# jrnerupudinho/Semi-Blind-Channel-Estimation-for-MIMO-RIS-communication-system-Using-EM-Algo

Measured on AMD Instinct MI355X. Metric: EM-iterations/sec (whole node) + NMSE@SNR; Nt=Nr=4, N_RIS=64, Tp=16 Td=256, higher is better.
Workload: dtype f64; 1 GPU; cfg1; n_tx=4, n_rx=4, N_RIS=64, T_p=16, T_d=256, M=16, trials_per_gpu=1000, em_iters=20, estep=soft, partition_r=0, solve=chol, parallelism=trials-sharded x1, streams_per_gpu=3

## Files before the change

semi-blind-channel-estimation-for-mimo-ris-communication-system-using-em-algo_amd/csrc/api.hip:

```cpp
#include <stdlib.h>
#include <string.h>

#include <atomic>
#include <initializer_list>
#include <mutex>
#include <vector>

#include "sbce_internal.h"

using namespace sbce;

namespace sbce {

#if SBCE_AB
DebugConfig g_debug;

namespace {
void read_debug_env(DebugConfig& c) {
    c = kDebugDefault;
    auto env = [](const char* n) { const char* v = getenv(n); return (v && v[0]) ? v : nullptr; };
    const char* v;
    if ((v = env("SBCE_ESTEP_IMPL"))) c.estep_valu = v[0] == 'v';
    if ((v = env("SBCE_ESTEP_PRUNE"))) c.estep_noprune = v[0] == '0';
    if ((v = env("SBCE_ESTEP_COUNT"))) c.estep_count = v[0] == '1';
    if ((v = env("SBCE_ESTEP_F32"))) c.estep_nof32 = v[0] == '0';
    if ((v = env("SBCE_ESTEP_SPHERE"))) c.estep_nosphere = v[0] == '0';
    if ((v = env("SBCE_SPHERE_BUDGET"))) {
        const int bu = atoi(v);
        c.sphere_budget = bu < 1 ? 1 : (bu > kBfsPmax ? kBfsPmax : bu);
    }
    if ((v = env("SBCE_BACKSUB"))) c.backsub_general = v[0] == '1';
    if ((v = env("SBCE_CHOL_IMPL"))) c.chol_valu = v[0] == 'v';
    if ((v = env("SBCE_ESTEP_PAIR"))) c.estep_nopair = v[0] == '0';
    if ((v = env("SBCE_CPLX3"))) c.cplx3 = v[0] != '0';
    if ((v = env("SBCE_MSTEP_SMALL"))) {
        c.mstep_nosmall = v[0] == '0';
        c.small_valu = v[0] == 'v';
        c.small_v1 = v[0] == '1';
    }
    if ((v = env("SBCE_PM_IMPL"))) c.pm_impl = (v[0] == 'w' || v[0] == 't' || v[0] == 'q') ? v[0] : 0;
    if ((v = env("SBCE_SMALL_SOLVE"))) c.small_col = v[0] == 'c';
    if ((v = env("SBCE_ESTEP_TRI"))) c.estep_tri = (v[0] >= '0' && v[0] <= '2') ? v[0] - '0' : 1;
    if ((v = env("SBCE_SMALL_STOP"))) c.small_stop = (v[0] >= '1' && v[0] <= '4') ? v[0] - '0' : 0;
}

__attribute__((constructor)) void load_debug_env() { read_debug_env(g_debug); }
}

bool debug_nondefault() {
    const DebugConfig& c = g_debug;
    const DebugConfig& d = kDebugDefault;
    return c.estep_valu != d.estep_valu || c.estep_noprune != d.estep_noprune ||
           c.estep_nof32 != d.estep_nof32 || c.estep_tri != d.estep_tri ||
           c.estep_nosphere != d.estep_nosphere || c.sphere_budget != d.sphere_budget ||
           c.backsub_general != d.backsub_general || c.chol_valu != d.chol_valu ||
           c.estep_nopair != d.estep_nopair || c.cplx3 != d.cplx3 ||
           c.mstep_nosmall != d.mstep_nosmall || c.small_stop != d.small_stop ||
           c.small_valu != d.small_valu || c.small_v1 != d.small_v1 || c.small_col != d.small_col ||
           (chol_debug_skip_mask() & 31);
}
#else
bool debug_nondefault() { return false; }
#endif

}

namespace {

constexpr size_t kAlign = 256;
size_t align_up(size_t v) { return (v + kAlign - 1) / kAlign * kAlign; }

struct Carve {
    size_t mom, R, rhs, done, mchg, ysh, prep, list, tree, tol, winv, ppsi, pS, pflag, prhs, gram, grhs,
        act, tol2, dvec, mnr, mnskip, total;
    bool has_prep, has_prhs, has_winv, has_mn;
};

constexpr int kAnySolve = -1;

bool make_problem(const sbce_dims* d, Problem& pb) {
    if (!d) return false;
    if (d->batch < 0 || d->n_tx < 1 || d->n_rx < 1 || d->n_psi < 1 || d->t_p < 0 || d->t_d < 1 ||
        d->m < 2 || d->partition_r < 0 || !(d->varn > 0.0))
        return false;
    if (d->n_tx > 8 || d->n_rx > 8) return false;
    pb.B = d->batch; pb.NT = d->n_tx; pb.NR = d->n_rx; pb.P = d->n_psi;
    pb.Tp = d->t_p; pb.Td = d->t_d; pb.M = d->m; pb.varn = d->varn; pb.pr = d->partition_r;
    pb.varx = d->varx;
    pb.L = pb.P * pb.NT;
    pb.K = pb.L * pb.NR;
    return true;
}

Carve carve(const Problem& pb, int solve = kAnySolve) {
    Carve c;
    const size_t MS = (size_t)pb.NT + (size_t)pb.NT * pb.NT;
    c.mom = 0;
    c.R = align_up(c.mom + (size_t)pb.B * pb.Td * MS * sizeof(cd));
    c.rhs = align_up(c.R + (size_t)pb.B * pb.L * pb.L * sizeof(cd));
    c.done = align_up(c.rhs + (size_t)pb.B * pb.L * pb.NR * sizeof(cd));
    c.ysh = align_up(c.done + (size_t)pb.B * sizeof(int32_t));
    c.mchg = c.ysh;
    c.prep = align_up(c.ysh + (size_t)pb.B * pb.Td * pb.NR * sizeof(cd));
    const int ps = estep_prep_stride(pb);
    c.has_prep = ps > 0;
    c.list = align_up(c.prep + (size_t)pb.B * pb.Td * ps * sizeof(double));
    c.tree = align_up(c.list + (3 * (size_t)pb.B * pb.Td + 2 * kEstepListCnt) * sizeof(int32_t));
    c.tol = c.has_prep ? align_up(c.tree + (size_t)pb.B * pb.Td * kTreeRecDoubles * sizeof(double))
                       : c.list;
    c.ppsi = c.pS = c.pflag = c.winv = c.tol;
    c.total = c.tol;
    if (rbuild_herm_supported(pb)) {
        c.ppsi = c.total;
        c.pS = align_up(c.ppsi + (size_t)pb.B * pb.Tp * pb.P * sizeof(cd));
        c.pflag = align_up(c.pS + (size_t)pb.B * pb.Tp * pb.NT * pb.NT * sizeof(cd));
        c.total = align_up(c.pflag + (size_t)pb.B * sizeof(int32_t));
    }
    c.has_prhs = rbuild_herm_supported(pb) && pb.L <= kLargeL;
    c.prhs = c.total;
    if (c.has_prhs) c.total = align_up(c.prhs + (size_t)pb.B * pb.L * pb.NR * sizeof(cd));
    c.tol = c.total;
    c.winv = align_up(c.tol + (size_t)pb.B * sizeof(double));
    c.total = c.winv;
    c.has_mn = solve == kAnySolve || solve == SBCE_SOLVE_MINNORM;
    c.has_winv = c.has_mn || pb.L > kLargeL;
    c.gram = c.winv;
    if (c.has_winv) c.total = c.gram = align_up(c.winv + (size_t)pb.B * 64 * 64 * sizeof(cd));
    c.grhs = c.act = c.tol2 = c.dvec = c.mnr = c.mnskip = c.total;
    if (c.has_mn) {
        c.grhs = align_up(c.gram + (size_t)pb.B * pb.L * pb.L * sizeof(cd));
        c.act = align_up(c.grhs + (size_t)pb.B * pb.L * pb.NR * sizeof(cd));
        c.tol2 = align_up(c.act + (size_t)pb.B * sizeof(int32_t));
        c.dvec = align_up(c.tol2 + (size_t)pb.B * sizeof(double));
        c.mnr = align_up(c.dvec + (size_t)pb.B * pb.L * sizeof(double));
        c.mnskip = align_up(c.mnr + (size_t)pb.B * pb.L * pb.NR * sizeof(cd));
        c.total = align_up(c.mnskip + (size_t)pb.B * sizeof(int32_t));
// ... 926 lines not shown
```

semi-blind-channel-estimation-for-mimo-ris-communication-system-using-em-algo_amd/csrc/estep_sweep.hip:

```cpp
#include "sbce_internal.h"

namespace sbce {

namespace {


template <int NT, int NR>
__device__ double candidate_distance(const cd* H, const cd* yg, const cd* s_cons, int M,
                                     double reg, cd* scratch, int lane, double& scale) {
    cd* sG = scratch;
    cd* sHy = scratch + 16;
    if (lane < NT * NT) {
        const int u = lane / NT, v = lane - u * NT;
        cd acc = czero();
#pragma unroll
        for (int r = 0; r < NR; ++r) acc = cfmac(acc, H[v * NR + r], H[u * NR + r]);
        if (u == v) acc.x += reg;
        sG[lane] = acc;
    } else if (lane >= 32 && lane < 32 + NT) {
        const int u = lane - 32;
        cd acc = czero();
#pragma unroll
        for (int r = 0; r < NR; ++r) acc = cfmac(acc, yg[r], H[u * NR + r]);
        sHy[u] = acc;
// ... 19 lines not shown
    }
#pragma unroll
    for (int i = 0; i < NT; ++i) {
        cd s = sHy[i];
#pragma unroll
        for (int k = 0; k < i; ++k) s = csub(s, cmul(Lm[i][k], z[k]));
        z[i] = cscale(s, dinv[i]);
    }
#pragma unroll
    for (int i = NT - 1; i >= 0; --i) {
        cd s = z[i];
#pragma unroll
        for (int k = i + 1; k < NT; ++k) s = csub(s, cmul(cconj(Lm[k][i]), z[k]));
        z[i] = cscale(s, dinv[i]);
    }
    const int qa = lane >> 4;
    cd za = z[0];
#pragma unroll
    for (int q = 1; q < NT; ++q) za = csel(qa == q, z[q], za);
    double bd = INFINITY;
    int bs = 0;
    if (qa < NT)
        for (int s = lane & 15; s < M; s += 16) {
            const double dd = cabs2(csub(za, s_cons[s]));
            if (dd < bd) { bd = dd; bs = s; }
        }
    for (int off = 8; off >= 1; off >>= 1) {
        const double od = shfl_xor_d(bd, off);
        const int os = __shfl_xor(bs, off);
        if (od < bd || (od == bd && os < bs)) { bd = od; bs = os; }
    }
    cd x[NT];
#pragma unroll
    for (int q = 0; q < NT; ++q) x[q] = s_cons[__shfl(bs, 16 * q)];
    double d0 = 0.0, sc = 0.0;
#pragma unroll
    for (int r = 0; r < NR; ++r) {
        cd res = yg[r];
        sc += cabs2(res);
#pragma unroll
        for (int q = 0; q < NT; ++q) {
            const cd hx = cmul(H[q * NR + r], x[q]);
            res = csub(res, hx);
            sc += NT * cabs2(hx);
        }
        d0 += cabs2(res);
    }
    wave_sync();
    scale = sc;
    return d0;
}


constexpr int kMfmaWaves = 2;
constexpr int kChunk = 256;
constexpr int kScreenD = 256;

typedef float f4v __attribute__((ext_vector_type(4)));

constexpr int mfma_rec_d(int rec_words) { return 2 * (rec_words <= 128 ? 160 : (rec_words + 1) / 2 * 2 + 32); }
constexpr int mfma_tri_d(int steps) { return 3 * 64 * steps / 2 + 128; }
constexpr int mfma_tab_d(int NO, int chunk, int steps, int M, int nkt_pad, int rec_words) {
    return (2 * NO + chunk + 3 * (4 * steps) * M + nkt_pad + 128 + 1) / 2 * 2 + mfma_rec_d(rec_words) +
           kScreenD + (M == 16 && chunk == 256 ? mfma_tri_d(steps) : 0);
}
constexpr int kTriGate = 4;

struct MfmaConst {
    int B, Td, P, M, lm;
    int JA, JB, chunk, nparts;
    int tab_d;
    double inv_s2, thr_d;
    double reg;
    int nkt_pad;
    int prune;
    int count;
    int prep_stride;
    int rowb_off;
    int rowb;
    int rec_words;
    int spw;
    int screen;
    int tri;
};

template <int NT, int NR>
__device__ double column_tile_bounds(const cd* H, const cd* yg, const cd* s_cons, int M, int lm,
                                     int nkt, double* s_lb, cd* scratch, int lane) {
    constexpr int NA = NT / 2, NB = NT - NA;
    const int mask = M - 1;
    const int r = lane & 7;
    const bool own = r < NR;
    int xa[6];
#pragma unroll
    for (int i = 0; i < 6; ++i) xa[i] = (lane ^ (32 >> i)) << 2;
    auto rsum = [&](double v) {
#pragma unroll
        for (int i = 3; i < 6; ++i) v += bperm_d(v, xa[i]);
        return v;
    };
    auto rdot = [&](cd u, cd v) { return cmk(rsum(fma(v.x, u.x, v.y * u.y)),
                                             rsum(fma(v.y, u.x, -v.x * u.y))); };
    cd u[NA];
    bool ok = true;
#pragma unroll
    for (int q = 0; q < NA; ++q) {
        cd v = own ? H[q * NR + r] : czero();
        const double h2 = rsum(cabs2(v));
#pragma unroll
        for (int rep = 0; rep < 2; ++rep)
#pragma unroll
            for (int j = 0; j < q; ++j) v = csub(v, cmul(u[j], rdot(u[j], v)));
        const double n2 = rsum(cabs2(v));
        ok = ok && h2 > 0.0 && n2 > 1e-6 * h2;
        u[q] = cscale(v, ok ? fast_rsqrt(n2) : 0.0);
    }
    cd w = own ? yg[r] : czero();
    double sc = rsum(cabs2(w));
    cd g[NB];
    double g2 = 0.0;
#pragma unroll
    for (int b = 0; b < NB; ++b) {
        g[b] = own ? H[(NA + b) * NR + r] : czero();
        g2 += cabs2(g[b]);
    }
#pragma unroll
    for (int j = 0; j < NA; ++j) {
        w = csub(w, cmul(u[j], rdot(u[j], w)));
#pragma unroll
        for (int b = 0; b < NB; ++b) g[b] = csub(g[b], cmul(u[j], rdot(u[j], g[b])));
    }
    if (lane < NR) {
        scratch[r] = w;
#pragma unroll
        for (int b = 0; b < NB; ++b) scratch[8 * (b + 1) + r] = g[b];
    }
    double cmax2 = lane < M ? cabs2(s_cons[lane]) : 0.0;
#pragma unroll
    for (int i = 0; i < 6; ++i) cmax2 = fmax(cmax2, bperm_d(cmax2, xa[i]));
    sc += NB * cmax2 * rsum(g2);
    wave_sync();
    for (int kt0 = 0; kt0 < nkt; kt0 += 4) {
        const int kt = kt0 + (lane >> 4);
        const int k = kt * 16 + (lane & 15);
        cd xb[NB];
#pragma unroll
        for (int b = 0; b < NB; ++b) xb[b] = s_cons[(k >> (lm * (NB - 1 - b))) & mask];
        double lb = 0.0;
#pragma unroll
        for (int rr = 0; rr < NR; ++rr) {
            cd res = scratch[rr];
#pragma unroll
            for (int b = 0; b < NB; ++b) res = csub(res, cmul(scratch[8 * (b + 1) + rr], xb[b]));
            lb += cabs2(res);
        }
        if (!ok) lb = 0.0;
#pragma unroll
        for (int i = 2; i < 6; ++i) lb = fmin(lb, bperm_d(lb, xa[i]));
        if ((lane & 15) == 0 && kt < nkt) s_lb[kt] = lb;
    }
    wave_sync();
    return sc;
}

__device__ unsigned long long g_estep_mfma;
__device__ unsigned long long g_estep_groups;
// ... 284 lines not shown
        for (int pass = 0; pass < 2; ++pass) {
            const int q = pass ? 1 : 3, o = pass ? 3 : 1;
            const cd hq = own ? H[q * NR + r] : czero();
            const cd v = own ? (vi == 0 ? yv[r] : H[(vi == 1 ? 0 : (vi == 2 ? o : 2)) * NR + r]) : czero();
            const double hq2 = rsum(cabs2(hq));
            const bool ok = range_ok && hq2 > 0.0 && hq2 >= 1e-20 * hmax;
            if (!__all(ok)) continue;
            const cd cf = cscale(cmk(rsum(fma(hq.x, v.x, hq.y * v.y)), rsum(fma(hq.x, v.y, -hq.y * v.x))),
                                 1.0 / hq2);
            const cd pvv = csub(v, cmul(hq, cf));
            wave_sync();
            if (lane < 32) pv[vi * 8 + r] = own ? pvv : czero();
            wave_sync();
            double uu = 0.0, vv = 0.0, qq = 0.0;
#pragma unroll
            for (int it = 0; it < STEPS; ++it) {
                const int kk = 4 * it + rq, e = kk * 16 + col;
                double u = 0.0, w = 0.0, q2 = 0.0;
                if (kk < K2) {
                    const int rr = kk >> 1;
                    const cd x = s_cons[col];
                    const cd pu = csub(pv[rr], cmul(pv[8 + rr], x));
                    const cd hv = cmul(pv[16 + rr], x);
                    const cd hx = cmul(pv[24 + rr], x);
                    u = -2.0 * ((kk & 1) ? pu.y : pu.x);
                    w = 2.0 * ((kk & 1) ? hv.y : hv.x);
                    q2 = (kk & 1) ? hx.y : hx.x;
                }
                tU[e] = (float)u;
                tV[e] = (float)w;
                tQ[e] = (float)q2;
                uu = fma(u, u, uu);
                vv = fma(w, w, vv);
                qq = fma(q2, q2, qq);
            }
            uu += bperm_d(uu, xaddr16); uu += bperm_d(uu, xaddr32);
            vv += bperm_d(vv, xaddr16); vv += bperm_d(vv, xaddr32);
            qq += bperm_d(qq, xaddr16); qq += bperm_d(qq, xaddr32);
            const double amaxp = 0.5 * (wave_max_dpp(uu) + wave_max_dpp(vv));
            const double margin = fma(0x1p-16, 2.0 * amaxp + qq, 1e-9 * S);
            wave_sync();
            float vr32[STEPS], qr32[STEPS];
            f4v cx = {0.f, 0.f, 0.f, 0.f};
#pragma unroll
            for (int s = 0; s < STEPS; ++s) {
                vr32[s] = tV[(4 * s + rq) * 16 + col];
                qr32[s] = tQ[(4 * s + rq) * 16 + col];
                cx = __builtin_amdgcn_mfma_f32_16x16x4f32(tU[(4 * s + rq) * 16 + col], vr32[s], cx, 0, 0, 0);
            }
#pragma unroll
            for (int j = 0; j < 4; ++j) {
                const double us = bperm_d(uu, (4 * rq + j) << 2);
                tA[(4 * rq + j) * 16 + col] = (float)fma(0.5, (double)cx[j], 0.25 * (us + vv));
            }
            wave_sync();
            double tq = 0.0;
#pragma unroll 1
            for (int blk = 0; blk < 4; ++blk) {
                f4v t[4];
#pragma unroll
                for (int u = 0; u < 4; ++u)
                    t[u] = *reinterpret_cast<const f4v*>(tA + (4 * blk + u) * 16 + rq * 4);
#pragma unroll
                for (int s = 0; s < STEPS; ++s)
#pragma unroll
                    for (int u = 0; u < 4; ++u)
                        t[u] = __builtin_amdgcn_mfma_f32_16x16x4f32(
                            tU[(4 * s + rq) * 16 + 4 * blk + u] + vr32[s], qr32[s], t[u], 0, 0, 0);
                float mm = fminf(fminf(t[0][0], t[0][1]), fminf(t[0][2], t[0][3]));
#pragma unroll
                for (int u = 1; u < 4; ++u)
                    mm = fminf(mm, fminf(fminf(t[u][0], t[u][1]), fminf(t[u][2], t[u][3])));
                mm = fminf(mm, __int_as_float(__builtin_amdgcn_ds_bpermute(xaddr16, __float_as_int(mm))));
                mm = fminf(mm, __int_as_float(__builtin_amdgcn_ds_bpermute(xaddr32, __float_as_int(mm))));
                if (rq == blk) tq = ((double)mm + qq) - margin;
            }
            tri_lane = fmax(tri_lane, tq);
        }
    };

    const double hard_bound = d0 + 1e-10 * cscale_d + 1e-300;
    unsigned groups = 0;
    unsigned reached = 0;
    unsigned long long ktmask = ~0ull;
    if (nktile <= 64) {
        const double lim0 = ((MODE == SBCE_ESTEP_HARD) ? hard_bound : mshift + thr_d) + lb_margin;
        ktmask = __ballot(lane < nktile && !(lbp[lane < nktile ? lane : 0] > lim0));
    }
    for (int kt = 0; kt < nktile; ++kt) {
        if (nktile <= 64) {
            const unsigned long long m = ktmask >> kt;
            if (!m) break;
            kt += __builtin_ctzll(m);
        }
        if (lbp[kt] > ((MODE == SBCE_ESTEP_HARD) ? hard_bound : mshift + thr_d) + lb_margin)
            continue;
        unsigned rowmask = 0xffffu;
        if constexpr (V16) {
            if (c.tri && !tri_have && (c.tri == 2 || reached >= kTriGate)) {
                build_tri();
                tri_have = true;
            }
            if (tri_have) {
                const double lim = (MODE == SBCE_ESTEP_HARD) ? hard_bound : mshift + thr_d;
                const unsigned long long lv = __ballot(tri_lane <= lim) >> kt;
                if (!(lv & 0x0001000100010001ull)) continue;
                rowmask = ((lv & 1) ? 0x000fu : 0u) | ((lv >> 16 & 1) ? 0x00f0u : 0u) |
                          ((lv >> 32 & 1) ? 0x0f00u : 0u) | ((lv >> 48 & 1) ? 0xf000u : 0u);
            }
        }
        if (rowb) {
            double bnd = INFINITY;
            if (lane < 16) {
                const cd x0 = s_cons[lane];
                const double* rk = s_rk + 3 * kt;
                bnd = fma(cabs2(x0), s_tab[63], rk[0] - 2.0 * (x0.x * rk[1] + x0.y * rk[2]));
            }
            const double lim = ((MODE == SBCE_ESTEP_HARD) ? hard_bound : mshift + thr_d) + lb_margin;
            rowmask &= (unsigned)__ballot(bnd <= lim);
            if (!rowmask) continue;
        }
        const int k = kt * 16 + col;
        cd xb[NB];
#pragma unroll
        for (int bb = 0; bb < NB; ++bb) xb[bb] = s_cons[(k >> (k_lm * (NB - 1 - bb))) & mask];
        double bop[STEPS];
        float bop32[STEPS];
        double gam = 0.0;
        if constexpr (V16) {
#pragma unroll
            for (int s = 0; s < STEPS; ++s) {
                bop[s] = s_Q2[(4 * s + rq) * 16 + kt] + q3reg[s];
                gam = fma(bop[s], bop[s], gam);
            }
            gam += bperm_d(gam, xaddr16);
            gam += bperm_d(gam, xaddr32);
#pragma unroll
            for (int s = 0; s < STEPS; ++s) bop32[s] = (float)bop[s];
        } else {
            cd qv[NR];
#pragma unroll
            for (int r = 0; r < NR; ++r) {
                cd acc = czero();
#pragma unroll
                for (int bb = 0; bb < NB; ++bb) acc = cfma(acc, H[(NA + bb) * NR + r], xb[bb]);
                qv[r] = acc;
                gam += cabs2(acc);
            }
#pragma unroll
            for (int s = 0; s < STEPS; ++s) {
                const int kk = 4 * s + rq;
                double v = 0.0;
#pragma unroll
                for (int r = 0; r < NR; ++r) {
                    if (kk == 2 * r) v = qv[r].x;
                    if (kk == 2 * r + 1) v = qv[r].y;
                }
                bop[s] = v;
            }
        }
        double ck = 0.0;
        cd mu[NA];
#pragma unroll
        for (int q = 0; q < NA; ++q) mu[q] = czero();
        bool touched = false;
        double R1[4] = {0.0, 0.0, 0.0, 0.0}, N0 = 0.0;
        cd Q[4] = {czero(), czero(), czero(), czero()};

        for (int i0 = 0; i0 < k_JA; i0 += k_chunk) {
            if (!table_ready && V16) {
                wave_sync();
                double nrm = 0.0;
                const double* T = lane < 16 ? s_U : s_V;
#pragma unroll
                for (int kk = 0; kk < K2; ++kk) {
                    const double v = T[kk * 16 + (lane & 15)];
                    nrm = fma(v, v, nrm);
                }
                if (lane < 32) s_tab[lane] = nrm;
                mf4 cx = {0.0, 0.0, 0.0, 0.0};
#pragma unroll
                for (int s = 0; s < STEPS; ++s)
                    cx = __builtin_amdgcn_mfma_f64_16x16x4f64(s_U[(4 * s + rq) * 16 + col], vreg[s],
                                                              cx, 0, 0, 0);
                wave_sync();
                const double nvv = s_tab[16 + col];
                double am = 0.0;
#pragma unroll
                for (int j = 0; j < 4; ++j) {
                    const int s0 = rq + 4 * j;
                    const double al = 0.25 * (s_tab[s0] + nvv) + 0.5 * cx[j];
                    s_al[s0 * 16 + (col & 3) * 4 + (col >> 2)] = al;
                    s_al32[s0 * 16 + col] = (float)al;
                    am = fmax(am, al);
                }
                amax = wave_max_dpp(am);
                wave_sync();
                table_ready = true;
            }
            if (!table_ready) {
                wave_sync();
                for (int e = lane; e < k_chunk; e += 64) {
                    const int i = i0 + e;
                    const int su = (NA == 2) ? (i >> k_lm) : i;
                    const int sv = i & mask;
                    double al = 0.0;
#pragma unroll
                    for (int kk = 0; kk < K2; ++kk) {
                        double v = s_U[kk * k_M + su];
                        if (NA == 2) v += s_V[kk * k_M + sv];
                        al = fma(v, v, al);
                    }
                    s_al[e] = 0.25 * al;
                }
                wave_sync();
                table_ready = (k_JA == k_chunk);
            }
            for (int tg = 0; tg < ntile_chunk; tg += TU) {
                if (V16 && !((rowmask >> tg) & ((1u << TU) - 1u))) continue;
                if constexpr (V16) {
                    if (tri_have && !__any(lane_d(tri_lane, kt + 4 * tg) <=
                                           ((MODE == SBCE_ESTEP_HARD) ? best_d : mshift + thr_d)))
                        continue;
                }
                ++reached;
                if (V16 && scr_on) {
                    f4v s32[TU];
#pragma unroll
                    for (int u = 0; u < TU; ++u)
                        s32[u] = *reinterpret_cast<const f4v*>(s_al32 + (tg + u) * 16 + rq * 4);
#pragma unroll
                    for (int s = 0; s < STEPS; ++s)
#pragma unroll
                        for (int u = 0; u < TU; ++u) {
                            const float av = s_U32[(4 * s + rq) * 16 + (i0 >> 4) + tg + u] + vreg32[s];
                            s32[u] = __builtin_amdgcn_mfma_f32_16x16x4f32(av, bop32[s], s32[u], 0, 0, 0);
                        }
                    float m32 = fminf(fminf(s32[0][0], s32[0][1]), fminf(s32[0][2], s32[0][3]));
#pragma unroll
                    for (int u = 1; u < TU; ++u)
                        m32 = fminf(m32, fminf(fminf(s32[u][0], s32[u][1]), fminf(s32[u][2], s32[u][3])));
                    const double lim = ((MODE == SBCE_ESTEP_HARD) ? best_d : mshift + thr_d) - gam +
                                       0x1p-17 * (2.0 * amax + gam);
                    ++scr_n;
                    const bool pass = __any((double)m32 <= lim);
                    scr_pass += pass;
                    if (scr_n >= 16 && 2 * scr_pass > scr_n) scr_on = false;
                    if (!pass) continue;
                }
                ++groups;
                mf4 acc[TU];
#pragma unroll
                for (int u = 0; u < TU; ++u) {
                    if (V16) {
                        const cd lo = *reinterpret_cast<const cd*>(s_al + (tg + u) * 16 + rq * 4);
                        const cd hi = *reinterpret_cast<const cd*>(s_al + (tg + u) * 16 + rq * 4 + 2);
                        acc[u] = mf4{lo.x, lo.y, hi.x, hi.y};
                    } else {
#pragma unroll
                        for (int j = 0; j < 4; ++j) acc[u][j] = s_al[(tg + u) * 16 + rq + 4 * j];
                    }
                }
#pragma unroll
                for (int s = 0; s < STEPS; ++s)
#pragma unroll
                    for (int u = 0; u < TU; ++u) {
                        const int kk = 4 * s + rq;
                        double av;
                        if (V16) {
                            av = s_U[kk * 16 + (i0 >> 4) + tg + u] + vreg[s];
                        } else {
                            const int ia = i0 + (tg + u) * 16 + col;
                            av = s_U[kk * k_M + ((NA == 2) ? (ia >> k_lm) : ia)];
                            if (NA == 2) av += s_V[kk * k_M + (ia & mask)];
                        }
                        acc[u] = __builtin_amdgcn_mfma_f64_16x16x4f64(av, bop[s], acc[u], 0, 0, 0);
                    }
                double cm = fmin(fmin(acc[0][0], acc[0][1]), fmin(acc[0][2], acc[0][3]));
#pragma unroll
                for (int u = 1; u < TU; ++u)
                    cm = fmin(cm, fmin(fmin(acc[u][0], acc[u][1]), fmin(acc[u][2], acc[u][3])));
                if (MODE == SBCE_ESTEP_HARD) {
                    if (!__any(cm + gam <= best_d)) continue;
                } else if (!__any(cm + gam <= mshift + thr_d)) {
                    continue;
                }
                if (MODE == SBCE_ESTEP_HARD) {
                    const double lim = best_d - gam;
#pragma unroll
                    for (int u = 0; u < TU; ++u)
#pragma unroll
                        for (int j = 0; j < 4; ++j) {
                            const double dv = acc[u][j];
                            if (dv <= lim) {
                                const int jj = (i0 + (tg + u) * 16 + rq + 4 * j) * k_JB + k;
                                const double dd = dv + gam;
                                if (dd < best_d || (dd == best_d && jj < best_j)) { best_d = dd; best_j = jj; }
                            }
                        }
                    continue;
                }
                cm += gam;
                if (__any(cm < mshift)) {
                    double mn = fmin(cm, mshift);
                    mn = wave_min_dpp(mn);
                    const double f = fexp_neg((mn - mshift) * inv_s2);
// ... 140 lines not shown
        for (int i = NV; i < 32; ++i) v[i] = 0.0;
#pragma unroll
        for (int st = 0; st < 5; ++st) {
            const int h = 16 >> st;
            const bool hi = (lane >> (5 - st)) & 1;
#pragma unroll
            for (int i = 0; i < h; ++i) {
                const double snd = hi ? v[i] : v[h + i];
                const double kp = hi ? v[h + i] : v[i];
                v[i] = kp + bperm_d(snd, xa[st]);
            }
        }
        v[0] += bperm_d(v[0], xa[5]);
        double* red = s_tab;
        const int j = ((lane >> 5) & 1) * 16 + ((lane >> 4) & 1) * 8 + ((lane >> 3) & 1) * 4 +
                      ((lane >> 2) & 1) * 2 + ((lane >> 1) & 1);
        wave_sync();
        if (!(lane & 1)) red[j] = v[0];
        wave_sync();
        if (lane < NT + NT * NT) {
            constexpr int OFF_KA = 1, OFF_KB = 1 + 2 * NPA;
            constexpr int BQ = 1 + 2 * NPA + 2 * NPB, SQ = 3 + 2 * NB;
            constexpr int BB = BQ + NA * SQ;
            int ire, iim = -1;
            bool cj = false;
            if (lane < NT) {
                ire = lane < NA ? BQ + lane * SQ : BB + 3 * (lane - NA);
                iim = ire + 1;
            } else {
                const int i = (lane - NT) / NT, j = (lane - NT) - (lane - NT) / NT * NT;
                if (i == j) {
                    ire = i < NA ? BQ + i * SQ + 2 : BB + 3 * (i - NA) + 2;
                } else if (i < NA && j < NA) {
                    ire = OFF_KA; iim = OFF_KA + 1; cj = i > j;
                } else if (i >= NA && j >= NA) {
                    ire = OFF_KB; iim = OFF_KB + 1; cj = i > j;
                } else if (i < NA) {
                    ire = BQ + i * SQ + 3 + 2 * (j - NA); iim = ire + 1;
                } else {
                    ire = BQ + j * SQ + 3 + 2 * (i - NA); iim = ire + 1; cj = true;
                }
            }
            const double iz = 1.0 / red[0];
            const double re = red[ire], im = iim >= 0 ? red[iim] : 0.0;
            const cd mv = mom_word(cmk(re * iz, (cj ? -im : im) * iz));
            out[lane] = mv;
            if (arm && mom_bits_differ(mold, mv)) a.mchg[b] = 1;
        }
    }
    }();
    }
    if (!listed) return;
    }
}

template <int NT, int NR, int MODE, int TU, bool V16 = false>
__global__ __launch_bounds__(128) void estep_mfma_kernel(EstepArgs a, MfmaConst c) {
    estep_mfma_body<NT, NR, MODE, TU, V16>(a, c);
}
bool make_mfma(const Problem& pb, MfmaConst& c, size_t& lds, long& blocks) {
    HypSplit h;
    if (!hyp_split(pb, h) || h.JA < 16 || h.JB < 16) return false;
    const long JA = h.JA, JB = h.JB;
    c.B = pb.B; c.Td = pb.Td; c.P = pb.P; c.M = pb.M; c.lm = h.lm;
    c.JA = (int)JA; c.JB = (int)JB;
    c.chunk = (int)(JA < kChunk ? JA : kChunk);
    const int NO = pb.NT * pb.NR;
    c.nparts = NO <= 64 ? 64 / NO : 1;
    const int steps = (2 * pb.NR + 3) / 4;
    c.nkt_pad = (int)((JB / 16 + 1) / 2 * 2);

    c.prune = !g_debug.estep_noprune;
    c.count = g_debug.estep_count;
    c.inv_s2 = 1.0 / (pb.varn * pb.varn);
    c.thr_d = kSkipThr * pb.varn * pb.varn;
    c.reg = 0.1 * pb.varn * pb.varn;
    c.rowb_off = 4 + 2 * NO + c.nkt_pad;
    c.prep_stride = c.rowb_off + (pb.NT == 4 ? 6 * pb.NR : 0);
    c.rec_words = c.prep_stride + 2 * pb.NR;
    c.tab_d = mfma_tab_d(NO, c.chunk, steps, pb.M, c.nkt_pad, c.rec_words);
    c.spw = 4;
    c.screen = !g_debug.estep_nof32;
    c.tri = g_debug.estep_tri;
    c.rowb = pb.NT == 4 && c.prune;
    lds = 64 * sizeof(cd) + (size_t)kMfmaWaves * c.tab_d * sizeof(double);
    const long nsym = (long)pb.B * pb.Td;
    const long per_block = (long)kMfmaWaves * c.spw;
    blocks = (nsym + per_block - 1) / per_block;
    return lds <= 160 * 1024;
}

template <int NT, int NR>
hipError_t dispatch_mfma_mode(const MfmaConst& c, size_t lds, long blocks, const EstepArgs& a,
                              int mode, hipStream_t s) {
    const bool tu4 = (c.chunk / 16) % 4 == 0;
    if constexpr (NT == 4) {
        if (c.M == 16 && tu4) {
            if (c.JA != 256 || c.JB != 256 || c.chunk != 256 || c.nkt_pad != 16 ||
                c.prep_stride != 4 + 2 * NT * NR + 16 + 6 * NR)
                return hipErrorInvalidValue;
            if (mode == SBCE_ESTEP_HARD)
                hipLaunchKernelGGL((estep_mfma_kernel<NT, NR, SBCE_ESTEP_HARD, 4, true>),
                                   dim3((unsigned)blocks), dim3(64 * kMfmaWaves), lds, s, a, c);
            else
                hipLaunchKernelGGL((estep_mfma_kernel<NT, NR, SBCE_ESTEP_SOFT, 4, true>),
                                   dim3((unsigned)blocks), dim3(64 * kMfmaWaves), lds, s, a, c);
            return hipGetLastError();
        }
    }
    if (mode == SBCE_ESTEP_HARD) {
        if (tu4)
            hipLaunchKernelGGL((estep_mfma_kernel<NT, NR, SBCE_ESTEP_HARD, 4>), dim3((unsigned)blocks),
                               dim3(64 * kMfmaWaves), lds, s, a, c);
        else
            hipLaunchKernelGGL((estep_mfma_kernel<NT, NR, SBCE_ESTEP_HARD, 1>), dim3((unsigned)blocks),
                               dim3(64 * kMfmaWaves), lds, s, a, c);
    } else {
        if (tu4)
            hipLaunchKernelGGL((estep_mfma_kernel<NT, NR, SBCE_ESTEP_SOFT, 4>), dim3((unsigned)blocks),
                               dim3(64 * kMfmaWaves), lds, s, a, c);
        else
            hipLaunchKernelGGL((estep_mfma_kernel<NT, NR, SBCE_ESTEP_SOFT, 1>), dim3((unsigned)blocks),
                               dim3(64 * kMfmaWaves), lds, s, a, c);
    }
    return hipGetLastError();
}

template <int NT>
hipError_t dispatch_mfma_nr(int NR, const MfmaConst& c, size_t lds, long blocks,
                            const EstepArgs& a, int mode, hipStream_t s) {
    switch (NR) {
        case 1: return dispatch_mfma_mode<NT, 1>(c, lds, blocks, a, mode, s);
        case 2: return dispatch_mfma_mode<NT, 2>(c, lds, blocks, a, mode, s);
        case 3: return dispatch_mfma_mode<NT, 3>(c, lds, blocks, a, mode, s);
        case 4: return dispatch_mfma_mode<NT, 4>(c, lds, blocks, a, mode, s);
        case 5: return dispatch_mfma_mode<NT, 5>(c, lds, blocks, a, mode, s);
        case 6: return dispatch_mfma_mode<NT, 6>(c, lds, blocks, a, mode, s);
        case 7: return dispatch_mfma_mode<NT, 7>(c, lds, blocks, a, mode, s);
        case 8: return dispatch_mfma_mode<NT, 8>(c, lds, blocks, a, mode, s);
    }
    return hipErrorInvalidValue;
}

}

hipError_t estep_debug_mfma(unsigned long long* out, int reset) {
    if (reset) {
        const unsigned long long z = 0;
        return hipMemcpyToSymbol(HIP_SYMBOL(g_estep_mfma), &z, sizeof(z), 0, hipMemcpyHostToDevice);
    }
    return hipMemcpyFromSymbol(out, HIP_SYMBOL(g_estep_mfma), sizeof(*out), 0,
                               hipMemcpyDeviceToHost);
}

hipError_t estep_debug_groups(unsigned long long* out, int reset) {
    if (reset) {
        const unsigned long long z = 0;
        return hipMemcpyToSymbol(HIP_SYMBOL(g_estep_groups), &z, sizeof(z), 0, hipMemcpyHostToDevice);
    }
    return hipMemcpyFromSymbol(out, HIP_SYMBOL(g_estep_groups), sizeof(*out), 0,
                               hipMemcpyDeviceToHost);
}

SweepPlan estep_sweep_plan(const Problem& pb) {
    MfmaConst c;
    size_t lds;
// ... 23 lines not shown
```

semi-blind-channel-estimation-for-mimo-ris-communication-system-using-em-algo_amd/csrc/sbce_internal.h:

```cpp
#pragma once

#include <hip/hip_runtime.h>
#include <stdint.h>
#include <math.h>

#include "../../include/sbce.h"

namespace sbce {

typedef double2 cd;

typedef double mf4 __attribute__((ext_vector_type(4)));
__device__ __forceinline__ mf4 mfma4(double a, double b, mf4 c) {
    return __builtin_amdgcn_mfma_f64_16x16x4f64(a, b, c, 0, 0, 0);
}
template <bool G3>
__device__ __forceinline__ void csub_init(mf4& cre, mf4& cim, mf4& c2) {
    c2 = mf4{0.0, 0.0, 0.0, 0.0};
    if constexpr (G3) cim += cre;
}
template <bool G3>
__device__ __forceinline__ void csub_step(mf4& cre, mf4& cim, mf4& c2, cd v, cd t) {
    if constexpr (G3) {
        cre = __builtin_amdgcn_mfma_f64_16x16x4f64(-v.x, t.x, cre, 0, 0, 0);
// ... 103 lines not shown
    argmin_step<0x141>(d, i);
    argmin_step<0x140>(d, i);
    double bd = lane_d(d, 0);
    int bi = __builtin_amdgcn_readlane(i, 0);
#pragma unroll
    for (int r = 16; r < 64; r += 16) {
        const double od = lane_d(d, r);
        const int oi = __builtin_amdgcn_readlane(i, r);
        if (od < bd || (od == bd && oi < bi)) { bd = od; bi = oi; }
    }
    d = bd;
    i = bi;
}
__device__ __forceinline__ double wave_min_dpp(double v) {
    v = fmin(v, dpp_d<0xB1>(v));
    v = fmin(v, dpp_d<0x4E>(v));
    v = fmin(v, dpp_d<0x141>(v));
    v = fmin(v, dpp_d<0x140>(v));
    return fmin(fmin(lane_d(v, 0), lane_d(v, 16)), fmin(lane_d(v, 32), lane_d(v, 48)));
}
__device__ __forceinline__ double wave_max_dpp(double v) {
    v = fmax(v, dpp_d<0xB1>(v));
    v = fmax(v, dpp_d<0x4E>(v));
    v = fmax(v, dpp_d<0x141>(v));
    v = fmax(v, dpp_d<0x140>(v));
    return fmax(fmax(lane_d(v, 0), lane_d(v, 16)), fmax(lane_d(v, 32), lane_d(v, 48)));
}
__device__ __forceinline__ double block_sum4(double v, double* red, int lane, int w) {
    if (lane == 0) red[w] = v;
    __syncthreads();
    return ((red[0] + red[1]) + red[2]) + red[3];
}
__device__ __forceinline__ double uniform_d(double v) {
    return __hiloint2double(__builtin_amdgcn_readfirstlane(__double2hiint(v)),
                            __builtin_amdgcn_readfirstlane(__double2loint(v)));
}
__device__ __forceinline__ double bperm_d(double v, int addr) {
    const int lo = __builtin_amdgcn_ds_bpermute(addr, __double2loint(v));
    const int hi = __builtin_amdgcn_ds_bpermute(addr, __double2hiint(v));
    return __hiloint2double(hi, lo);
}

__device__ __forceinline__ double fast_rsqrt(double x) {
    const int e = __builtin_amdgcn_frexp_exp(x);
    const int h = e >> 1;
    const double xs = __builtin_amdgcn_ldexp(x, -2 * h);
    double y = (double)__builtin_amdgcn_rsqf((float)xs);
    double r = fma(-xs * y, y, 1.0);
    y = fma(0.5 * y, r, y);
    r = fma(-xs * y, y, 1.0);
    y = fma(0.5 * y, r, y);
    return __builtin_amdgcn_ldexp(y, -h);
}
__device__ __forceinline__ double fast_rsqrt64(double x) {
    double y = __builtin_amdgcn_rsq(x);
    double r = fma(-x * y, y, 1.0);
    y = fma(0.5 * y, r, y);
    r = fma(-x * y, y, 1.0);
    return fma(0.5 * y, r, y);
}


#ifndef SBCE_AB
#define SBCE_AB 0
#endif
struct DebugConfig {
    bool estep_valu;
    bool estep_noprune;
    bool estep_count;
    bool estep_nof32;
    bool estep_nosphere;
    int sphere_budget;
    bool backsub_general;
    bool chol_valu;
    bool estep_nopair;
    bool cplx3;
    bool mstep_nosmall;
    bool small_valu;
    bool small_v1;
    int small_stop;
    bool small_col;
    char pm_impl;
    int estep_tri;
};
inline constexpr DebugConfig kDebugDefault = {false, false, false, false, false, 128, false, false,
                                              false, true, false, false, false, 0, false, 0, 1};
#if SBCE_AB
extern DebugConfig g_debug;
#else
inline constexpr DebugConfig g_debug = kDebugDefault;
#endif
bool debug_nondefault();

struct Problem {
    int B, NT, NR, P, Tp, Td, M, L, K;
    int pr;
    double varn;
    double varx;
};

struct EstepArgs {
    const cd* yd;
    const cd* psid;
    const cd* theta;
    const cd* cons;
    cd* mom;
    const int32_t* done;
    int32_t* status;
    double* prep;
    int32_t* list;
    double* tree;
    const double* varn_t = nullptr;
    bool lists_zeroed = false;
    int32_t* mchg = nullptr;
};

__device__ __forceinline__ unsigned mom_bits_differ(const cd& u, const cd& v) {
    const unsigned long long d = ((unsigned long long)__double_as_longlong(u.x) ^
                                  (unsigned long long)__double_as_longlong(v.x)) |
                                 ((unsigned long long)__double_as_longlong(u.y) ^
                                  (unsigned long long)__double_as_longlong(v.y));
    return (unsigned)(d | (d >> 32));
}
__device__ __forceinline__ cd mom_word(const cd& v) { return cmk(v.x + 0.0, v.y + 0.0); }
__device__ __forceinline__ void mom_store(cd* p, const cd& v, bool arm, unsigned& chg) {
    if (arm) chg |= mom_bits_differ(*p, v);
    *p = v;
}

constexpr double kSkipThr = 50.0;
struct TrialNoise {
    double inv_s2, thr_d, reg, s2;
};
__device__ __forceinline__ TrialNoise trial_noise(double v) {
    TrialNoise n;
    n.inv_s2 = 1.0 / (v * v);
    n.thr_d = kSkipThr * v * v;
    n.reg = 0.1 * v * v;
    n.s2 = v * v;
    return n;
}
struct GridLds {
    double lre[8], lim[8];
    int idx[64];
    int K;
};

__device__ inline void grid_build(const cd* cons, int M, GridLds* g) {
    const int tid = threadIdx.x;
    int K = 0;
    while (K * K < M) ++K;
    const bool sq = K * K == M && K <= 8;
    bool ok = true;
    if (sq && tid < M) {
        const cd v = cons[tid];
        int lt_x = 0, eq_x = 0, lt_y = 0, eq_y = 0, same = 0;
        for (int s = 0; s < M; ++s) {
            const cd u = cons[s];
            lt_x += u.x < v.x;
            eq_x += u.x == v.x;
            lt_y += u.y < v.y;
            eq_y += u.y == v.y;
            same += (u.x == v.x) && (u.y == v.y);
        }
        ok = eq_x == K && eq_y == K && same == 1 && lt_x % K == 0 && lt_y % K == 0;
        if (ok) {
            const int ir = lt_x / K, ii = lt_y / K;
            g->lre[ir] = v.x;
            g->lim[ii] = v.y;
// ... 320 lines not shown
```

Baseline: 1.429 million EM-iterations/s.

## Visit E-step candidate tiles in ascending lower-bound order with early break

In the soft E-step sweep, the column tiles are sorted by their lower bounds using a per-lane rank and a DPP OR-reduction, then visited best-first, and the loop breaks at the first tile whose bound exceeds the threshold. Within each tile, the four row blocks are also reordered by their row bound. The intent is to tighten the running minimum (mshift) sooner, so that more tiles and blocks get pruned. This adds ranking work per symbol, and the ordered break assumes the lower bounds stay monotone against a threshold that may move. Screening counters are also adjusted.

```diff
diff --git a/semi-blind-channel-estimation-for-mimo-ris-communication-system-using-em-algo_amd/csrc/api.hip b/semi-blind-channel-estimation-for-mimo-ris-communication-system-using-em-algo_amd/csrc/api.hip
--- a/semi-blind-channel-estimation-for-mimo-ris-communication-system-using-em-algo_amd/csrc/api.hip
+++ b/semi-blind-channel-estimation-for-mimo-ris-communication-system-using-em-algo_amd/csrc/api.hip
@@ -41,6 +41,7 @@
     if ((v = env("SBCE_PM_IMPL"))) c.pm_impl = (v[0] == 'w' || v[0] == 't' || v[0] == 'q') ? v[0] : 0;
     if ((v = env("SBCE_SMALL_SOLVE"))) c.small_col = v[0] == 'c';
     if ((v = env("SBCE_ESTEP_TRI"))) c.estep_tri = (v[0] >= '0' && v[0] <= '2') ? v[0] - '0' : 1;
+    if ((v = env("SBCE_ESTEP_ORDER"))) c.estep_noorder = v[0] == '0';
     if ((v = env("SBCE_SMALL_STOP"))) c.small_stop = (v[0] >= '1' && v[0] <= '4') ? v[0] - '0' : 0;
 }
 
@@ -51,7 +52,7 @@
     const DebugConfig& c = g_debug;
     const DebugConfig& d = kDebugDefault;
     return c.estep_valu != d.estep_valu || c.estep_noprune != d.estep_noprune ||
-           c.estep_nof32 != d.estep_nof32 || c.estep_tri != d.estep_tri ||
+           c.estep_nof32 != d.estep_nof32 || c.estep_tri != d.estep_tri || c.estep_noorder != d.estep_noorder ||
            c.estep_nosphere != d.estep_nosphere || c.sphere_budget != d.sphere_budget ||
            c.backsub_general != d.backsub_general || c.chol_valu != d.chol_valu ||
            c.estep_nopair != d.estep_nopair || c.cplx3 != d.cplx3 ||
diff --git a/semi-blind-channel-estimation-for-mimo-ris-communication-system-using-em-algo_amd/csrc/estep_sweep.hip b/semi-blind-channel-estimation-for-mimo-ris-communication-system-using-em-algo_amd/csrc/estep_sweep.hip
--- a/semi-blind-channel-estimation-for-mimo-ris-communication-system-using-em-algo_amd/csrc/estep_sweep.hip
+++ b/semi-blind-channel-estimation-for-mimo-ris-communication-system-using-em-algo_amd/csrc/estep_sweep.hip
@@ -125,6 +125,7 @@
     int spw;
     int screen;
     int tri;
+    int order;
 };
 
 template <int NT, int NR>
@@ -575,20 +576,53 @@
     const double hard_bound = d0 + 1e-10 * cscale_d + 1e-300;
     unsigned groups = 0;
     unsigned reached = 0;
-    unsigned long long ktmask = ~0ull;
-    if (nktile <= 64) {
+    constexpr bool ORD = V16 && MODE != SBCE_ESTEP_HARD;
+    const bool ordered = ORD && (SBCE_AB ? c.order != 0 : true);
+    unsigned long long ktord = 0xfedcba9876543210ull;
+    if constexpr (ORD) {
+        if (ordered) {
+            const double lbc = lbp[col];
+            const double mine = lbc < lb_margin ? 0.0 : lbc;
+            int rank = 0;
+#pragma unroll
+            for (int j = 0; j < 16; ++j) {
+                const double lbj = lbp[j];
+                const double o = lbj < lb_margin ? 0.0 : lbj;
+                rank += (o < mine || (o == mine && j < col)) ? 1 : 0;
+            }
+            const unsigned nib = (unsigned)col << ((rank & 7) << 2);
+            unsigned lo = rank < 8 ? nib : 0u, hi = rank < 8 ? 0u : nib;
+            auto row_or = [](unsigned v) {
+                v |= (unsigned)__builtin_amdgcn_update_dpp(0, (int)v, 0xB1, 0xF, 0xF, false);
+                v |= (unsigned)__builtin_amdgcn_update_dpp(0, (int)v, 0x4E, 0xF, 0xF, false);
+                v |= (unsigned)__builtin_amdgcn_update_dpp(0, (int)v, 0x141, 0xF, 0xF, false);
+                v |= (unsigned)__builtin_amdgcn_update_dpp(0, (int)v, 0x140, 0xF, 0xF, false);
+                return (unsigned)__builtin_amdgcn_readfirstlane((int)v);
+            };
+            lo = row_or(lo);
+            hi = row_or(hi);
+            ktord = ((unsigned long long)hi << 32) | lo;
+        }
+    }
+    [[maybe_unused]] unsigned long long ktmask = ~0ull;
+    if (!ORD && nktile <= 64) {
         const double lim0 = ((MODE == SBCE_ESTEP_HARD) ? hard_bound : mshift + thr_d) + lb_margin;
         ktmask = __ballot(lane < nktile && !(lbp[lane < nktile ? lane : 0] > lim0));
     }
-    for (int kt = 0; kt < nktile; ++kt) {
-        if (nktile <= 64) {
+    for (int kt = 0, kn = 0; (ORD ? kn : kt) < nktile; ++kt, ++kn) {
+        if constexpr (ORD) {
+            kt = (int)(ktord >> (4 * kn)) & 15;
+        } else if (nktile <= 64) {
             const unsigned long long m = ktmask >> kt;
             if (!m) break;
             kt += __builtin_ctzll(m);
         }
-        if (lbp[kt] > ((MODE == SBCE_ESTEP_HARD) ? hard_bound : mshift + thr_d) + lb_margin)
+        if (lbp[kt] > ((MODE == SBCE_ESTEP_HARD) ? hard_bound : mshift + thr_d) + lb_margin) {
+            if (ORD && ordered) break;
             continue;
+        }
         unsigned rowmask = 0xffffu;
+        [[maybe_unused]] unsigned blkord = 0xe4u;
         if constexpr (V16) {
             if (c.tri && !tri_have && (c.tri == 2 || reached >= kTriGate)) {
                 build_tri();
@@ -597,21 +631,46 @@
             if (tri_have) {
                 const double lim = (MODE == SBCE_ESTEP_HARD) ? hard_bound : mshift + thr_d;
                 const unsigned long long lv = __ballot(tri_lane <= lim) >> kt;
-                if (!(lv & 0x0001000100010001ull)) continue;
                 rowmask = ((lv & 1) ? 0x000fu : 0u) | ((lv >> 16 & 1) ? 0x00f0u : 0u) |
                           ((lv >> 32 & 1) ? 0x0f00u : 0u) | ((lv >> 48 & 1) ? 0xf000u : 0u);
             }
         }
+        unsigned rowlive = 0xffffu;
+        double bnd = INFINITY;
         if (rowb) {
-            double bnd = INFINITY;
             if (lane < 16) {
                 const cd x0 = s_cons[lane];
                 const double* rk = s_rk + 3 * kt;
                 bnd = fma(cabs2(x0), s_tab[63], rk[0] - 2.0 * (x0.x * rk[1] + x0.y * rk[2]));
             }
             const double lim = ((MODE == SBCE_ESTEP_HARD) ? hard_bound : mshift + thr_d) + lb_margin;
-            rowmask &= (unsigned)__ballot(bnd <= lim);
-            if (!rowmask) continue;
+            rowlive = (unsigned)__ballot(bnd <= lim);
+        }
+        if constexpr (V16) {
+            if (tri_have && scr_on) {
+                unsigned rl = rowlive | (rowlive >> 1);
+                rl |= rl >> 2;
+                scr_n += __builtin_popcount(rl & ~rowmask & 0x1111u);
+            }
+        }
+        rowmask &= rowlive;
+        if (!rowmask) continue;
+        if constexpr (ORD) {
+            if (rowb && ordered) {
+                double bm = fmin(bnd, dpp_d<0xB1>(bnd));
+                bm = fmin(bm, dpp_d<0x4E>(bm));
+                bm = bm < lb_margin ? 0.0 : bm;
+                const int blk = (lane >> 2) & 3;
+                int rank = 0;
+#pragma unroll
+                for (int j = 0; j < 4; ++j) {
+                    const double o = lane_d(bm, 4 * j);
+                    rank += (o < bm || (o == bm && j < blk)) ? 1 : 0;
+                }
+                const int code = blk << (2 * rank);
+                blkord = (unsigned)(__builtin_amdgcn_readlane(code, 0) | __builtin_amdgcn_readlane(code, 4) |
+                                    __builtin_amdgcn_readlane(code, 8) | __builtin_amdgcn_readlane(code, 12));
+            }
         }
         const int k = kt * 16 + col;
         cd xb[NB];
@@ -709,12 +768,14 @@
                 wave_sync();
                 table_ready = (k_JA == k_chunk);
             }
-            for (int tg = 0; tg < ntile_chunk; tg += TU) {
+            for (int tg = 0, tn = 0; (ORD ? tn : tg) < ntile_chunk; tg += TU, tn += TU) {
+                if constexpr (ORD) tg = (int)((blkord >> (tn >> 1)) & 3u) << 2;
                 if (V16 && !((rowmask >> tg) & ((1u << TU) - 1u))) continue;
                 if constexpr (V16) {
-                    if (tri_have && !__any(lane_d(tri_lane, kt + 4 * tg) <=
-                                           ((MODE == SBCE_ESTEP_HARD) ? best_d : mshift + thr_d)))
-                        continue;
+                    const bool dead = tri_have && !__any(lane_d(tri_lane, kt + 4 * tg) <=
+                                                         ((MODE == SBCE_ESTEP_HARD) ? best_d : mshift + thr_d));
+                    scr_n += (int)(dead & scr_on);
+                    if (dead) continue;
                 }
                 ++reached;
                 if (V16 && scr_on) {
@@ -1021,6 +1082,7 @@
     c.spw = 4;
     c.screen = !g_debug.estep_nof32;
     c.tri = g_debug.estep_tri;
+    c.order = !g_debug.estep_noorder;
     c.rowb = pb.NT == 4 && c.prune;
     lds = 64 * sizeof(cd) + (size_t)kMfmaWaves * c.tab_d * sizeof(double);
     const long nsym = (long)pb.B * pb.Td;
diff --git a/semi-blind-channel-estimation-for-mimo-ris-communication-system-using-em-algo_amd/csrc/sbce_internal.h b/semi-blind-channel-estimation-for-mimo-ris-communication-system-using-em-algo_amd/csrc/sbce_internal.h
--- a/semi-blind-channel-estimation-for-mimo-ris-communication-system-using-em-algo_amd/csrc/sbce_internal.h
+++ b/semi-blind-channel-estimation-for-mimo-ris-communication-system-using-em-algo_amd/csrc/sbce_internal.h
@@ -209,9 +209,10 @@
     bool small_col;
     char pm_impl;
     int estep_tri;
+    bool estep_noorder;
 };
 inline constexpr DebugConfig kDebugDefault = {false, false, false, false, false, 128, false, false,
-                                              false, true, false, false, false, 0, false, 0, 1};
+                                              false, true, false, false, false, 0, false, 0, 1, false};
 #if SBCE_AB
 extern DebugConfig g_debug;
 #else
```

Result: faster. 1.515 million EM-iterations/s (median of 6 runs) (+6.1%).
